# bergmanlab/TELR

Hardware: AMD Instinct MI355X
Metric: gbp_aligned_per_s (higher is better)
Workload: dtype int16

## Files before the change

telr_amd/csrc/kernels.hip.h:

```cpp
#pragma once
#include <hip/hip_runtime.h>
#include <stdint.h>

#define TELR_NEG      (-(1 << 28))
#include "part_plan.h"
#define SK_TILE       1024
#define SK_THREADS    256
#define DP_DMAX       4096

struct ChainOpt {
    int32_t max_gap, bw, min_cnt, min_chain_score, chain_gap_q8, chain_skip_q8;
    int32_t dense_n, dense_span, mw_n;
};
struct DpOpt {
    int32_t a, b, q, e, q2, e2, sc_ambi, zdrop;
    int32_t cx_scale, cx_open, cx_emax, cx_emin, cx_dec, cx_flat;
};
__host__ __device__ __forceinline__ int d_cx_ext(const DpOpt &o, int len) { int v = o.cx_emax - o.cx_dec * len; return v > o.cx_emin ? v : o.cx_emin; }
__host__ __device__ __forceinline__ int d_cx_cost(const DpOpt &o, int L)
{
    int t = o.cx_open;
    for (int i = 0; i < L && i < o.cx_flat; ++i) t += d_cx_ext(o, i);
    if (L > o.cx_flat) t += (L - o.cx_flat) * o.cx_emin;
    return t;
// ... 367 lines not shown
            const int x = __ffsll((long long)f) - 1; f &= f - 1;
            s_code[o] = (uint8_t)d_chunk_base(C, x); s_start[o] = (uint32_t)(p0 + x); ++o;
        }
    }
    __syncthreads();
    const int n = o_end - o_first;
    for (int z = threadIdx.x; z < n; z += 128) { hstart[o_first + z] = s_start[z]; hcode[o_first + z] = s_code[z]; }
}
__global__ void k_hpc_seq_offsets(const int64_t *__restrict__ boff, int32_t sid0, int32_t nseq, int64_t chunk0, const int32_t *__restrict__ coff,
                                  int32_t nchunk, int32_t total, int32_t *__restrict__ hoff )
{
    const int s = blockIdx.x * blockDim.x + threadIdx.x;
    if (s > nseq) return;
    if (s == nseq) { hoff[s] = total; return; }
    const int64_t c = boff[sid0 + s] / 64 - chunk0;
    hoff[s] = c < nchunk ? coff[c] : total;
}

struct SketchHpcArgs {
    const uint8_t *hcode; const uint32_t *hstart;
    const int32_t *hoff;
    const int32_t *len;
    const uint32_t *goff;
    const int32_t *tile_seq, *tile_u0;
    int32_t k, w;
    int32_t *tile_cnt; const int32_t *tile_off;
    uint64_t *out_x; uint32_t *out_y;
};

template <int MODE>
__global__ void __launch_bounds__(SK_THREADS) k_sketch_hpc(SketchHpcArgs A)
{
    extern __shared__ __align__(16) unsigned char smem[];
    const int halo = A.w - 1, nslot = SK_TILE + 2 * halo, k = A.k;
    uint64_t *xs = (uint64_t*)smem;
    uint32_t *ps = (uint32_t*)(xs + nslot);
    uint8_t *cb = (uint8_t*)(ps + nslot);
    uint32_t *cw = (uint32_t*)(cb + ((nslot + k - 1 + 3) & ~3)), *cn = cw + (nslot + k - 1 + 15) / 16 + 3;
    __shared__ int32_t wsum[SK_THREADS / 64];
    const int t = blockIdx.x, tid = threadIdx.x;
    const int sid = A.tile_seq[t], u0 = A.tile_u0[t];
    const int h0 = A.hoff[sid], nh = A.hoff[sid + 1] - h0, ns = nh - k + 1, L = A.len[sid];
    const uint64_t mask = (1ULL << 2 * k) - 1;
    const int lo = u0 - halo;
    for (int s = tid; s < nslot + k - 1; s += SK_THREADS) { int r = lo + s; cb[s] = (r >= 0 && r < nh) ? A.hcode[h0 + r] : 4; }
    __syncthreads();
    const int ncode = nslot + k - 1;
    for (int wq = tid; wq < (ncode + 15) / 16 + 3; wq += SK_THREADS) {
        uint32_t v = 0;
        for (int z = 0; z < 16; ++z) { const int q = wq * 16 + z; if (q < ncode) v |= (uint32_t)(cb[q] & 3) << (2 * z); }
        cw[wq] = v;
    }
    for (int wq = tid; wq < (ncode + 31) / 32 + 2; wq += SK_THREADS) {
        uint32_t v = 0;
        for (int z = 0; z < 32; ++z) { const int q = wq * 32 + z; if (q >= ncode || cb[q] > 3) v |= 1u << z; }
        cn[wq] = v;
    }
    __syncthreads();
    for (int s = tid; s < nslot; s += SK_THREADS) {
        const int u = lo + s;
        uint64_t x = UINT64_MAX; uint32_t pz = 0;
        if (u >= 0 && u < ns) {
            const int wi = s >> 4, sh = (s & 15) * 2;
            const uint64_t lo64 = (uint64_t)cw[wi] | (uint64_t)cw[wi + 1] << 32, hi64 = cw[wi + 2];
            uint64_t v = lo64 >> sh;
            if (sh) v |= hi64 << (64 - sh);
            v &= mask;
            const uint64_t nb = (((uint64_t)cn[s >> 5] | (uint64_t)cn[(s >> 5) + 1] << 32) >> (s & 31)) & ((1ULL << k) - 1);
            const bool ok = nb == 0;
            const uint64_t fw = d_rev2(v, k), rv = (~v) & mask;
            const uint32_t first = A.hstart[h0 + u];
            const uint32_t last = (u + k < nh ? A.hstart[h0 + u + k] : (uint32_t)L) - 1;
            const uint32_t span = last - first + 1;
            if (ok && fw != rv && span < 256) {
                const uint32_t z = fw < rv ? 0 : 1;
                x = d_hash64(z ? rv : fw, mask) << 8 | (uint64_t)span;
                pz = last << 1 | z;
            }
        }
        xs[s] = x; ps[s] = pz;
    }
    __syncthreads();
    const int need = A.w < ns ? A.w : ns;
    uint32_t sel = 0;
#pragma unroll
    for (int c = 0; c < SK_TILE / SK_THREADS; ++c) {
        int s = halo + tid * (SK_TILE / SK_THREADS) + c, u = lo + s;
        uint64_t x = xs[s];
        const bool is_mz = halo == 9 ? d_mz_selected<9, uint64_t>(xs, s, u, ns, need, halo, x) : d_mz_selected<0, uint64_t>(xs, s, u, ns, need, halo, x);
        if (u < ns && x != UINT64_MAX && is_mz) sel |= 1u << c;
    }
    int cnt = __popc(sel);
    int lane = tid & 63, wv = tid >> 6, inc = cnt;
#pragma unroll
    for (int o = 1; o < 64; o <<= 1) { int v = __shfl_up(inc, o); if (lane >= o) inc += v; }
    if (lane == 63) wsum[wv] = inc;
    __syncthreads();
    int wbase = 0, total = 0;
#pragma unroll
    for (int i = 0; i < SK_THREADS / 64; ++i) { if (i < wv) wbase += wsum[i]; total += wsum[i]; }
    if (MODE == 0 || MODE == 2) {
        if (tid == 0) A.tile_cnt[t] = total;
    }
    if (MODE != 0) {
        int64_t o = (MODE == 2 ? (int64_t)t * SK_TILE : (int64_t)A.tile_off[t]) + wbase + inc - cnt;
        const uint32_t g0 = A.goff ? A.goff[sid] : 0u;
#pragma unroll
        for (int c = 0; c < SK_TILE / SK_THREADS; ++c) if (sel >> c & 1) {
            int s = halo + tid * (SK_TILE / SK_THREADS) + c;
            A.out_x[o] = xs[s];
            A.out_y[o] = ((g0 << 1) + ps[s]);
            ++o;
        }
    }
}

__global__ void __launch_bounds__(256) k_ix_hash_keys(const uint64_t *__restrict__ x, const uint32_t *__restrict__ y, int64_t n, uint64_t *__restrict__ key, uint32_t *__restrict__ val)
{
    const int64_t i = (int64_t)blockIdx.x * blockDim.x + threadIdx.x;
    if (i >= n) return;
    key[i] = x[i] >> 8;
    if (val != y) val[i] = y[i];
}
__global__ void k_head_flags(const uint64_t *__restrict__ h, int64_t n, int32_t *__restrict__ flag)
{
    int64_t i = (int64_t)blockIdx.x * blockDim.x + threadIdx.x;
    if (i < n) flag[i] = (i == 0 || h[i] != h[i - 1]) ? 1 : 0;
}
__global__ void k_write_entries(const uint64_t *__restrict__ h, const int32_t *__restrict__ flag, const int32_t *__restrict__ rank,
                                int64_t n, uint64_t *__restrict__ ent_hash, uint32_t *__restrict__ ent_off, int32_t n_ent)
{
    int64_t i = (int64_t)blockIdx.x * blockDim.x + threadIdx.x;
    if (i < n && flag[i]) { ent_hash[rank[i]] = h[i]; ent_off[rank[i]] = (uint32_t)i; }
    if (i == 0) ent_off[n_ent] = (uint32_t)n;
}
__global__ void k_ent_counts(const uint32_t *__restrict__ ent_off, int32_t n_ent, uint32_t *__restrict__ cnt)
{
    int32_t i = blockIdx.x * blockDim.x + threadIdx.x;
    if (i < n_ent) cnt[i] = ent_off[i + 1] - ent_off[i];
}
__device__ __forceinline__ uint32_t d_ht_slot(uint64_t h, int ht_shift, uint32_t ht_mask)
{
    return (uint32_t)((h * 0x9E3779B97F4A7C15ULL) >> ht_shift) & ht_mask;
}
#ifndef HT_FB_LOG
#define HT_FB_LOG 1
#endif
__device__ __forceinline__ uint32_t d_ht_filter_bit(uint64_t h, int ht_shift) { return (uint32_t)((h * 0x9E3779B97F4A7C15ULL) >> (ht_shift - HT_FB_LOG)); }
struct HtSlot { uint64_t hash; uint32_t off, cnt; };
#define HT_EMPTY 0xffffffffffffffffULL
struct IndexView {
    const uint64_t *ent_hash; const uint32_t *ent_off; const uint32_t *pos; const uint32_t *bstart;
    const uint32_t *goff; const int32_t *tlen;
    int32_t n_ent; int32_t shift; int32_t k, w;
    const HtSlot *ht; int32_t ht_shift; uint32_t ht_mask;
    const uint32_t *ht_home;
};
__global__ void k_ht_build(const uint64_t *__restrict__ ent_hash, const uint32_t *__restrict__ ent_off, int32_t n_ent, int ht_shift, uint32_t ht_mask, HtSlot *__restrict__ ht,
                           uint32_t *__restrict__ ht_home, const uint32_t *__restrict__ pos)
{
    const int e = blockIdx.x * blockDim.x + threadIdx.x;
    if (e >= n_ent) return;
    const uint64_t h = ent_hash[e];
    uint32_t s = d_ht_slot(h, ht_shift, ht_mask);
    { const uint32_t f = d_ht_filter_bit(h, ht_shift); atomicOr(&ht_home[f >> 5], 1u << (f & 31)); }
    for (;;) {
        const unsigned long long old = atomicCAS((unsigned long long*)&ht[s].hash, (unsigned long long)HT_EMPTY, (unsigned long long)h);
        if (old == HT_EMPTY) { const uint32_t c = ent_off[e + 1] - ent_off[e]; ht[s].off = c == 1 ? pos[ent_off[e]] : ent_off[e]; ht[s].cnt = c; return; }
        s = (s + 1) & ht_mask;
    }
}
template <bool FILTER = true>
__device__ __forceinline__ bool d_ht_lookup(const IndexView &I, uint64_t h, uint32_t &off, uint32_t &cnt)
{
    uint32_t s = d_ht_slot(h, I.ht_shift, I.ht_mask);
    if (FILTER) { const uint32_t f = d_ht_filter_bit(h, I.ht_shift); if (!((I.ht_home[f >> 5] >> (f & 31)) & 1u)) return false; }
    for (;;) {
        const uint4 v = *(const uint4*)&I.ht[s];
        const uint64_t hh = (uint64_t)v.y << 32 | v.x;
        if (hh == h) { off = v.z; cnt = v.w; return true; }
        if (hh == HT_EMPTY) return false;
        s = (s + 1) & I.ht_mask;
    }
}

__device__ __forceinline__ uint32_t d_wave_scan_add(uint32_t v)
{
    v += (uint32_t)__builtin_amdgcn_update_dpp(0, (int)v, 0x111, 0xf, 0xf, true);
    v += (uint32_t)__builtin_amdgcn_update_dpp(0, (int)v, 0x112, 0xf, 0xf, true);
    v += (uint32_t)__builtin_amdgcn_update_dpp(0, (int)v, 0x114, 0xf, 0xf, true);
    v += (uint32_t)__builtin_amdgcn_update_dpp(0, (int)v, 0x118, 0xf, 0xf, true);
    v += (uint32_t)__builtin_amdgcn_update_dpp(0, (int)v, 0x142, 0xa, 0xf, true);
    v += (uint32_t)__builtin_amdgcn_update_dpp(0, (int)v, 0x143, 0xc, 0xf, true);
    return v;
}

struct SeedArgs {
    IndexView I;
    const uint64_t *mz_x; const uint32_t *mz_y;
    const int32_t *q_mzoff;
    const int32_t *qlen;
    const int32_t *qtarget;
    const int32_t *q_order;
    int32_t mid_occ;
    const int32_t *tmid;
    int32_t per_target;
    int32_t n_targets;
    int32_t *mz_cnt;
    int32_t *mz_ent;
    int32_t *mz_n;
    int32_t *mz_aoff;
    int32_t *q_cnt;
    const int32_t *q_aoff;
    uint64_t *keys;
    const int32_t *tile_off, *q_tile0;
    uint64_t *lds_keys;
    int32_t rescue;
};

__device__ __forceinline__ void d_put_key(const SeedArgs &A, int64_t w, uint64_t key)
{
    if (A.lds_keys) A.lds_keys[w] = key; else A.keys[w] = key;
}
__device__ __forceinline__ int d_tid_of(const uint32_t *__restrict__ goff, int n, uint32_t g)
{
    int lo = 0, hi = n - 1;
    while (lo < hi) { const int mid = (lo + hi + 1) >> 1; if (goff[mid] <= g) lo = mid; else hi = mid - 1; }
    return lo;
}

__device__ __forceinline__ uint32_t d_occ_lower(const uint32_t *__restrict__ pos, uint32_t lo, uint32_t hi, uint32_t g)
{
    while (lo < hi) { const uint32_t mid = lo + ((hi - lo) >> 1); if ((pos[mid] >> 1) < g) lo = mid + 1; else hi = mid; }
    return lo;
}
#define SEED_RESCUE_DIST    500
#define SEED_RESCUE_MAX_OCC 4095
#define SEED_RESCUE_LIST    1024
__host__ __device__ __forceinline__ int32_t seed_rescue_k(int32_t pe, int32_t ps)
{
    return (int32_t)((1000LL * (pe - ps) + 249500LL) / 500000LL);
}
__device__ __forceinline__ int64_t d_mz_slot(const SeedArgs &A, int q, int g)
{
    if (!A.tile_off) return g;
    int lo = A.q_tile0[q], hi = A.q_tile0[q + 1] - 1;
    while (lo < hi) { const int mid = (lo + hi + 1) >> 1; if (A.tile_off[mid] <= g) lo = mid; else hi = mid - 1; }
    return (int64_t)lo * SK_TILE + (g - A.tile_off[lo]);
}
__device__ __forceinline__ uint64_t d_wave_min_u64(uint64_t v)
{
    for (int o = 32; o >= 1; o >>= 1) {
        const uint64_t u = (uint64_t)(uint32_t)__shfl_xor((int)(uint32_t)v, o) | (uint64_t)(uint32_t)__shfl_xor((int)(uint32_t)(v >> 32), o) << 32;
        v = u < v ? u : v;
    }
    return v;
}
__device__ __forceinline__ void d_seed_rescue(const SeedArgs &A, const int q, const int m0, const int m1, int32_t *__restrict__ mark, const int tid, const int nthr)
{
    __shared__ int32_t s_start[SEED_RESCUE_LIST];
    __shared__ int32_t s_nstart;
    const int32_t *__restrict__ occ = A.mz_n;
    const int32_t cut = A.mid_occ;
    const int lane = tid & 63, wv = __builtin_amdgcn_readfirstlane(tid >> 6), nwv = nthr >> 6;
    const int qlen = A.qlen[q];
    for (int gb = m0; gb < m1; gb += nthr) {
        if (tid == 0) s_nstart = 0;
        __syncthreads();
        const int g = gb + tid;
        if (g < m1 && occ[g] > cut && (g == m0 || occ[g - 1] <= cut)) s_start[atomicAdd(&s_nstart, 1)] = g;
        __syncthreads();
        const int ns = s_nstart;
        for (int si = wv; si < ns; si += nwv) {
            const int s = s_start[si];
            int e = s + 1;
            for (;;) {
                const int j = e + lane;
                const uint64_t stop = __ballot(j >= m1 || occ[j < m1 ? j : m1 - 1] <= cut);
                if (stop) { e += __builtin_ctzll(stop); break; }
                e += 64;
            }
            if (e > m1) e = m1;
            const int32_t ps = s > m0 ? (int32_t)(A.mz_y[d_mz_slot(A, q, s - 1)] >> 1) : 0;
            const int32_t pe = e < m1 ? (int32_t)(A.mz_y[d_mz_slot(A, q, e)] >> 1) : qlen;
            const int32_t k = seed_rescue_k(pe, ps);
            uint64_t last = 0; bool first = true;
            for (int z = 0; z < k; ++z) {
                uint64_t best = ~0ULL;
                for (int j = s + lane; j < e; j += 64) {
                    const int32_t c = occ[j];
                    const uint64_t key = (uint64_t)(uint32_t)c << 32 | (uint32_t)(j - s);
                    if (c < SEED_RESCUE_MAX_OCC && (first || key > last) && key < best) best = key;
                }
                best = d_wave_min_u64(best);
                if (best == ~0ULL) break;
                if (lane == 0) mark[s + (int32_t)(uint32_t)best] = (int32_t)(best >> 32);
                last = best; first = false;
            }
        }
        __syncthreads();
    }
}

template <int MODE>
__device__ __forceinline__ void d_seed_query(const SeedArgs &A, const int q, const int tid, const int nthr)
{
    const int m0 = A.q_mzoff[q], m1 = A.q_mzoff[q + 1];
    const int tf = A.qtarget ? A.qtarget[q] : -1;
    const bool pt = tf < 0 && A.per_target && A.tmid;
    uint32_t g0 = 0, g1 = 0xffffffffu;
    if (tf >= 0) { g0 = A.I.goff[tf]; g1 = g0 + (uint32_t)A.I.tlen[tf]; }
    const int32_t occ = (tf >= 0 && A.tmid) ? A.tmid[tf] : A.mid_occ;
    const int qlen = A.qlen[q];
    int t = A.tile_off ? A.q_tile0[q] : 0, t_lo = 0, t_hi = 0;
    if (A.tile_off) { t_lo = A.tile_off[t]; t_hi = A.tile_off[t + 1]; }
    const int64_t wbase = MODE == 1 && !A.lds_keys ? A.q_aoff[q] : 0;
    __shared__ int32_t s_wtot[16];
    int32_t carry = 0;
    for (int gb = m0; gb < m1; gb += nthr) {
      int32_t cnt_out = 0;
      const int g = gb + tid;
      if (g < m1) do {
        int64_t gi = g;
        if (A.tile_off) {
            while (g >= t_hi) { ++t; t_lo = t_hi; t_hi = A.tile_off[t + 1]; }
            gi = (int64_t)t * SK_TILE + (g - t_lo);
        }
        uint64_t x = A.mz_x[gi];
        uint32_t o0 = 0, o1 = 0;
        if (MODE == 0) {
            uint32_t off = 0, n = 0;
            if (!d_ht_lookup(A.I, x >> 8, off, n)) n = 0;
            A.mz_ent[g] = (int32_t)off; A.mz_n[g] = (int32_t)n;
            o0 = off; o1 = off + n;
        } else {
            if (A.mz_cnt[g] == 0) break;
            o0 = (uint32_t)A.mz_ent[g]; o1 = o0 + (uint32_t)A.mz_n[g];
        }
        const bool single = o1 - o0 == 1u;
        const uint32_t pos1 = o0;
#define SEED_POS(i_) (single ? pos1 : A.I.pos[i_])
        if (pt) {
            int32_t total = 0; int64_t w = MODE == 1 ? wbase + A.mz_aoff[g] : 0;
            uint64_t kf = 0, kr = 0; int32_t qz = 0;
            if (MODE == 1) {
                const uint32_t y = A.mz_y[gi];
                const int32_t span = (int32_t)(x & 0xff), qpos = (int32_t)(y >> 1); qz = (int32_t)(y & 1);
                kf = (uint64_t)qpos << 8 | (uint64_t)span;
                kr = (1ULL << 63) | (uint64_t)(qlen - (qpos + 1 - span) - 1) << 8 | (uint64_t)span;
            }
            uint32_t o = o0;
            while (o < o1) {
                const int t = d_tid_of(A.I.goff, A.n_targets, SEED_POS(o) >> 1);
                const uint32_t gend = A.I.goff[t + 1];
                uint32_t e = o + 1;
                for (int lin = 0; e < o1 && (SEED_POS(e) >> 1) < gend; ) { ++e; if (++lin == 8) { e = d_occ_lower(A.I.pos, e, o1, gend); break; } }
                if ((int32_t)(e - o) <= A.tmid[t]) {
                    total += (int32_t)(e - o);
                    if (MODE == 1) for (uint32_t z = o; z < e; ++z) { const uint32_t py = SEED_POS(z); d_put_key(A, w++, ((int)(py & 1) == qz ? kf : kr) | (uint64_t)(py >> 1) << 32); }
                }
                o = e;
            }
            cnt_out = total;
            break;
        }
        int32_t cnt = 0;
        uint32_t a0 = o0, a1 = o1;
        if (o1 > o0) {
            if (tf >= 0) {
                if (single) { const uint32_t gp = pos1 >> 1; if (gp < g0 || gp >= g1) a1 = a0; }
                else { a0 = d_occ_lower(A.I.pos, o0, o1, g0); a1 = d_occ_lower(A.I.pos, a0, o1, g1); }
            }
            cnt = (int32_t)(a1 - a0);
            if (cnt > occ && !(MODE == 1 && A.rescue && tf < 0)) cnt = 0;
        }
        cnt_out = cnt;
        if (MODE == 1 && cnt > 0) {
            uint32_t y = A.mz_y[gi];
            int32_t span = (int32_t)(x & 0xff), qpos = (int32_t)(y >> 1), qz = (int32_t)(y & 1);
            uint64_t kf = (uint64_t)qpos << 8 | (uint64_t)span;
            uint64_t kr = (1ULL << 63) | (uint64_t)(qlen - (qpos + 1 - span) - 1) << 8 | (uint64_t)span;
            int64_t w = wbase + A.mz_aoff[g];
            for (uint32_t o = a0; o < a1; ++o) {
                const uint32_t py = SEED_POS(o);
                d_put_key(A, w++, ((int)(py & 1) == qz ? kf : kr) | (uint64_t)(py >> 1) << 32);
            }
        }
      } while (0);
      if (MODE == 0 && g < m1) A.mz_cnt[g] = cnt_out;
    }
    if (MODE == 0) {
        __syncthreads();
        if constexpr (MODE == 0) { if (A.rescue && tf < 0) { d_seed_rescue(A, q, m0, m1, A.mz_cnt, tid, nthr); __syncthreads(); } }
        const int wv = tid >> 6, nwv = (nthr + 63) >> 6;
        for (int gb = m0; gb < m1; gb += nthr) {
            const int g = gb + tid;
            const int32_t c = g < m1 ? A.mz_cnt[g] : 0;
            const uint32_t inc = d_wave_scan_add((uint32_t)c);
            if ((tid & 63) == 63) s_wtot[wv] = (int32_t)inc;
            __syncthreads();
            int32_t before = 0, all = 0;
            for (int z = 0; z < nwv; ++z) { const int32_t v = s_wtot[z]; if (z < wv) before += v; all += v; }
            if (g < m1) A.mz_aoff[g] = carry + before + (int32_t)inc - c;
            carry += all;
            __syncthreads();
        }
        if (tid == 0) A.q_cnt[q] = carry;
    }
}
#undef SEED_POS
template <int MODE>
__global__ void __launch_bounds__(256) k_seed(SeedArgs A)
{
    d_seed_query<MODE>(A, A.q_order ? A.q_order[blockIdx.x] : blockIdx.x, threadIdx.x, blockDim.x);
}

#define VOTE_SLOTS   2048
#define VOTE_SUBCAP  512
#ifndef VOTE_WAVES
#define VOTE_WAVES   3
#endif
#ifndef VOTE_HCAP
#define VOTE_HCAP    768
#endif
#define VOTE_MZ      128
struct VoteOpt { int32_t len, shift, vmin, frac_q8; };
struct VoteArgs {
    const int64_t *q_soff;
    uint64_t *stage;
    int32_t *q_cnt;
};
__device__ __forceinline__ uint32_t d_vote_slot(uint32_t gp, uint32_t qadj, uint32_t rev, int shift)
{
    const uint32_t d = gp - qadj + (1u << 24);
    return (((d >> shift) & (VOTE_SLOTS / 2 - 1)) << 1) | rev;
}
template <bool FILTER>
__global__ void __launch_bounds__(256) k_vote_lookup(IndexView I, const uint64_t *__restrict__ mz_x, int32_t nmz, int32_t mid_occ, int32_t *__restrict__ mz_ent, int32_t *__restrict__ mz_n, int32_t rescue)
{
    const int g = blockIdx.x * 256 + threadIdx.x;
    if (g >= nmz) return;
    uint32_t off = 0, n = 0;
    if (!d_ht_lookup<FILTER>(I, mz_x[g] >> 8, off, n)) n = 0;
    if (n > (uint32_t)mid_occ && !rescue) n = 0;
    mz_ent[g] = (int32_t)off; mz_n[g] = (int32_t)n;
}
__global__ void __launch_bounds__(256) k_vote_rescue(SeedArgs A)
{
    const int q = blockIdx.x, tid = threadIdx.x;
    const int m0 = A.q_mzoff[q], m1 = A.q_mzoff[q + 1];
    for (int g = m0 + tid; g < m1; g += 256) A.mz_cnt[g] = 0;
    __syncthreads();
    d_seed_rescue(A, q, m0, m1, A.mz_cnt, tid, 256);
    __syncthreads();
    for (int g = m0 + tid; g < m1; g += 256) if (A.mz_n[g] > A.mid_occ) A.mz_n[g] = A.mz_cnt[g];
}
__global__ void __launch_bounds__(64) k_vote_qhits(const int32_t *__restrict__ q_mzoff, const int32_t *__restrict__ mz_n, int32_t nq, int64_t *__restrict__ q_hits)
{
    const int q = blockIdx.x, lane = threadIdx.x;
    if (q > nq) return;
    int64_t s = 0;
    if (q < nq) for (int g = q_mzoff[q] + lane; g < q_mzoff[q + 1]; g += 64) s += mz_n[g];
    for (int o = 32; o >= 1; o >>= 1) s += (int64_t)((uint64_t)(uint32_t)__shfl_xor((int)(uint32_t)s, o) | (uint64_t)(uint32_t)__shfl_xor((int)(uint32_t)((uint64_t)s >> 32), o) << 32);
    if (lane == 0) q_hits[q] = s;
}
#ifndef VOTE_WIN
#define VOTE_WIN 8
#endif
struct VoteChunk { uint32_t P[VOTE_MZ], off[VOTE_MZ], qpos[VOTE_MZ]; uint16_t zs[VOTE_MZ]; uint8_t rid[VOTE_MZ]; uint32_t wm[2 * VOTE_WIN]; };
struct VoteHit { uint32_t gp; uint32_t sm; };
template <bool T16> __device__ __forceinline__ uint32_t d_vt_add(uint32_t *T, uint32_t s)
{
    if (T16) { const uint32_t sh = (s & 1u) << 4; return ((atomicAdd(&T[s >> 1], 1u << sh) >> sh) & 0xffffu) + 1u; }
    return atomicAdd(&T[s], 1u) + 1u;
}
template <bool T16> __device__ __forceinline__ void d_vt_vote(uint32_t *T, uint32_t s)
{
    if (T16) (void)__hip_atomic_fetch_add(&T[s >> 1], 1u << ((s & 1u) << 4), __ATOMIC_RELAXED, __HIP_MEMORY_SCOPE_WORKGROUP);
    else (void)__hip_atomic_fetch_add(&T[s], 1u, __ATOMIC_RELAXED, __HIP_MEMORY_SCOPE_WORKGROUP);
}
template <bool T16> __device__ __forceinline__ uint32_t d_vt_get(const uint32_t *T, uint32_t s)
{
    return T16 ? (T[s >> 1] >> ((s & 1u) << 4)) & 0xffffu : T[s];
}
template <bool T16>
__global__ void __launch_bounds__(64 * VOTE_WAVES) k_seed_vote(SeedArgs A, VoteOpt V, VoteArgs VA, int64_t lim16)
{
    constexpr int TW = T16 ? VOTE_SLOTS / 2 : VOTE_SLOTS;
    {
        const int q_ = A.q_order ? A.q_order[blockIdx.x] : blockIdx.x;
        const bool small = VA.q_soff[q_ + 1] - VA.q_soff[q_] <= lim16;
        if (small != T16) return;
    }
    __shared__ uint32_t tab[VOTE_WAVES][TW];
    __shared__ VoteHit stash[VOTE_WAVES][VOTE_HCAP];
    __shared__ VoteChunk chunk[VOTE_WAVES];
    __shared__ int32_t sub_first[VOTE_SUBCAP + 1];
    __shared__ uint32_t blk_cnt;
    const int q = A.q_order ? A.q_order[blockIdx.x] : blockIdx.x;
    const int m0 = A.q_mzoff[q], m1 = A.q_mzoff[q + 1];
    const int qlen = A.qlen[q];
    const int tid = threadIdx.x, lane = tid & 63, wv = __builtin_amdgcn_readfirstlane(tid >> 6);
    uint32_t *T = tab[wv];
    VoteHit *HS = stash[wv];
    VoteChunk &C = chunk[wv];
    uint64_t *out = VA.stage + VA.q_soff[q];
    for (int i = lane; i < TW; i += 64) T[i] = 0;
    if (tid == 0) blk_cnt = 0;
    const int nsub = (qlen + V.len - 1) / V.len;
    for (int sb = 0; sb < nsub; sb += VOTE_SUBCAP) {
        __syncthreads();
        for (int i = tid; i <= VOTE_SUBCAP; i += 64 * VOTE_WAVES) sub_first[i] = m1;
        __syncthreads();
        for (int g = m0 + tid; g < m1; g += 64 * VOTE_WAVES) {
            const int s = (int)(A.mz_y[g] >> 1) / V.len;
            const int sp = g > m0 ? (int)(A.mz_y[g - 1] >> 1) / V.len : -1;
            if (s != sp) {
                int lo = sp + 1 > sb ? sp + 1 : sb, hi = s < sb + VOTE_SUBCAP ? s : sb + VOTE_SUBCAP;
                for (int j = lo; j <= hi; ++j) sub_first[j - sb] = g;
            }
        }
        __syncthreads();
        const int send = nsub < sb + VOTE_SUBCAP ? nsub : sb + VOTE_SUBCAP;
        uint32_t pf_off[2] = {0, 0}, pf_n[2] = {0, 0}, pf_y[2] = {0, 0}, pf_sp[2] = {0, 0}; int pf_s = -1;
#define VOTE_LOAD_CHUNK(o_, n_, y_, sp_, gc_, g1_) { _Pragma("unroll") for (int u = 0; u < 2; ++u) { const int g = (gc_) + 2 * lane + u; o_[u] = 0; n_[u] = 0; y_[u] = 0; sp_[u] = 0; \
            if (g < (g1_)) { o_[u] = (uint32_t)A.mz_ent[g]; n_[u] = (uint32_t)A.mz_n[g]; y_[u] = A.mz_y[g]; sp_[u] = ((const uint32_t*)A.mz_x)[2 * (size_t)g]; } } }
#define VOTE_PIN(o_, n_, y_, sp_) { _Pragma("unroll") for (int u = 0; u < 2; ++u) asm volatile("" : "+v"(o_[u]), "+v"(n_[u]), "+v"(y_[u]), "+v"(sp_[u])); }
        for (int s = sb + wv; s < send; s += VOTE_WAVES) {
            const int g0 = __builtin_amdgcn_readfirstlane(sub_first[s - sb]), g1 = __builtin_amdgcn_readfirstlane(sub_first[s - sb + 1]);
            uint32_t c0_off[2], c0_n[2], c0_y[2], c0_sp[2];
            if (pf_s == s) {
                VOTE_PIN(pf_off, pf_n, pf_y, pf_sp)
#pragma unroll
                for (int u = 0; u < 2; ++u) { c0_off[u] = pf_off[u]; c0_n[u] = pf_n[u]; c0_y[u] = pf_y[u]; c0_sp[u] = pf_sp[u]; }
            } else VOTE_LOAD_CHUNK(c0_off, c0_n, c0_y, c0_sp, g0, g1)
            if (s + VOTE_WAVES < send) { pf_s = s + VOTE_WAVES; const int pg0 = __builtin_amdgcn_readfirstlane(sub_first[pf_s - sb]), pg1 = __builtin_amdgcn_readfirstlane(sub_first[pf_s - sb + 1]); VOTE_LOAD_CHUNK(pf_off, pf_n, pf_y, pf_sp, pg0, pg1) }
            if (g0 >= g1) continue;
            uint32_t vmax = 0, nhit = 0;
            for (int pass = 0; pass < 2; ++pass) {
                if (pass == 1 && nhit <= VOTE_HCAP) break;
                uint32_t thr1 = 0;
                if (pass == 1) { thr1 = (vmax * (uint32_t)V.frac_q8 + 255u) >> 8; if (thr1 < (uint32_t)V.vmin) thr1 = (uint32_t)V.vmin; }
                uint32_t hbase = 0;
                for (int gc = g0; gc < g1; gc += VOTE_MZ) {
                    uint32_t n2[2];
                    __builtin_amdgcn_wave_barrier();
                    uint32_t c_off[2], c_y[2], c_sp[2];
                    if (gc == g0) {
#pragma unroll
                        for (int u = 0; u < 2; ++u) { c_off[u] = c0_off[u]; n2[u] = c0_n[u]; c_y[u] = c0_y[u]; c_sp[u] = c0_sp[u]; }
                    } else VOTE_LOAD_CHUNK(c_off, n2, c_y, c_sp, gc, g1)
#pragma unroll
                    for (int u = 0; u < 2; ++u) { C.qpos[2 * lane + u] = c_y[u] >> 1; C.zs[2 * lane + u] = (uint16_t)((c_y[u] & 1u) << 8 | (c_sp[u] & 0xffu)); }
                    uint32_t inc = n2[0] + n2[1];
                    inc = d_wave_scan_add(inc);
                    const uint64_t nz0 = __ballot(n2[0] > 0), nz1 = __ballot(n2[1] > 0);
                    const uint64_t below = (1ULL << lane) - 1ULL;
                    const uint32_t rk0 = (uint32_t)__popcll(nz0 & below) + (uint32_t)__popcll(nz1 & below);
                    if (n2[0]) { C.rid[rk0] = (uint8_t)(2 * lane); C.P[rk0] = inc - n2[1]; C.off[rk0] = c_off[0]; }
                    if (n2[1]) { const uint32_t rk1 = rk0 + (n2[0] ? 1u : 0u); C.rid[rk1] = (uint8_t)(2 * lane + 1); C.P[rk1] = inc; C.off[rk1] = c_off[1]; }
                    const uint32_t st0 = inc - n2[0] - n2[1], st1 = inc - n2[1];
                    uint32_t cb = 0;
                    __builtin_amdgcn_wave_barrier();
                    const uint32_t H = (uint32_t)__builtin_amdgcn_readlane((int)inc, 63);
                    for (uint32_t h0 = 0; h0 < H; h0 += 64 * VOTE_WIN) {
                        uint32_t m_[VOTE_WIN], py_[VOTE_WIN]; bool in_[VOTE_WIN];
                        if (lane < 2 * VOTE_WIN) C.wm[lane] = 0;
                        __builtin_amdgcn_wave_barrier();
                        { const uint32_t d0 = st0 - h0, d1 = st1 - h0;
                          if (n2[0] && d0 < 64u * VOTE_WIN) atomicOr(&C.wm[d0 >> 5], 1u << (d0 & 31));
                          if (n2[1] && d1 < 64u * VOTE_WIN) atomicOr(&C.wm[d1 >> 5], 1u << (d1 & 31)); }
                        __builtin_amdgcn_wave_barrier();
#pragma unroll
                        for (int u = 0; u < VOTE_WIN; ++u) {
                            const uint32_t h = h0 + 64 * u + lane;
                            in_[u] = h < H; m_[u] = 0; py_[u] = 0;
                            if (h0 + 64 * u < H) {
                                const uint64_t wmask = (uint64_t)C.wm[2 * u + 1] << 32 | C.wm[2 * u];
                                const uint32_t upto = (uint32_t)__popcll(wmask & ((2ULL << lane) - 1ULL));
                                if (in_[u]) {
                                    const uint32_t r = cb + upto - 1u;
                                    const uint32_t pm = r ? C.P[r - 1] : 0u, nm = C.P[r] - pm, of = C.off[r];
                                    m_[u] = C.rid[r];
                                    py_[u] = nm == 1 ? of : A.I.pos[of + (h - pm)];
                                }
                                cb += (uint32_t)__popcll(wmask);
                            }
                        }
#pragma unroll
                        for (int u = 0; u < VOTE_WIN; ++u) {
                            if (h0 + 64 * u >= H) break;
                            const uint32_t h = h0 + 64 * u + lane;
                            bool pass_hit = false; uint32_t gp_ = 0, rv_ = 0;
                            if (in_[u]) {
                                const uint32_t m = m_[u], zs = C.zs[m], span = zs & 0xffu, qpos = C.qpos[m];
                                rv_ = (py_[u] & 1u) ^ (zs >> 8); gp_ = py_[u] >> 1;
                                const uint32_t qadj = rv_ ? (uint32_t)qlen - (qpos + 1 - span) - 1 : qpos;
                                const uint32_t sl_ = d_vote_slot(gp_, qadj, rv_, V.shift);
                                if (pass == 0) {
                                    d_vt_vote<T16>(T, sl_);
                                    if (hbase + h < VOTE_HCAP) { VoteHit x; x.gp = gp_; x.sm = sl_ | m << 11 | (uint32_t)(gc - g0) / VOTE_MZ << 18; HS[hbase + h] = x; }
                                } else pass_hit = d_vt_get<T16>(T, (sl_ - 2u) & (VOTE_SLOTS - 1)) + d_vt_get<T16>(T, sl_) + d_vt_get<T16>(T, (sl_ + 2u) & (VOTE_SLOTS - 1)) >= thr1;
                            }
                            if (pass == 1) {
                                const uint64_t bm = __ballot(pass_hit);
                                uint32_t base = 0;
                                if (lane == 0 && bm) base = atomicAdd(&blk_cnt, (uint32_t)__popcll(bm));
                                base = (uint32_t)__shfl((int)base, 0);
                                if (pass_hit) {
                                    const uint32_t m = m_[u], zs = C.zs[m], span = zs & 0xffu, qpos = C.qpos[m];
                                    const uint64_t key = (rv_ ? (1ULL << 63) | (uint64_t)((uint32_t)qlen - (qpos + 1 - span) - 1) << 8 : (uint64_t)qpos << 8) | (uint64_t)span | (uint64_t)gp_ << 32;
                                    out[base + (uint32_t)__popcll(bm & ((1ULL << lane) - 1ULL))] = key;
                                }
                            }
                        }
                    }
                    hbase += H;
                }
                if (pass == 0) {
                    nhit = hbase;
                    if (nhit > VOTE_HCAP) {
                        __builtin_amdgcn_wave_barrier();
                        for (int i = lane; i < TW; i += 64) { const uint32_t w_ = T[i]; const uint32_t a_ = T16 ? (w_ & 0xffffu) : w_, b_ = T16 ? (w_ >> 16) : 0u; vmax = a_ > vmax ? a_ : vmax; vmax = b_ > vmax ? b_ : vmax; }
                        for (int o = 32; o >= 1; o >>= 1) { const uint32_t v = (uint32_t)__shfl_xor((int)vmax, o); vmax = v > vmax ? v : vmax; }
                    }
                }
            }
            __builtin_amdgcn_wave_barrier();
            const bool one_chunk = g1 - g0 <= VOTE_MZ;
            if (nhit <= VOTE_HCAP) {
                constexpr int NG = VOTE_HCAP / 64;
                VoteHit xs[NG]; uint32_t s3[NG]; uint32_t cmax = 0;
#pragma unroll
                for (int g = 0; g < NG; ++g) {
                    xs[g].gp = 0; xs[g].sm = 0; s3[g] = 0;
                    if ((uint32_t)(g * 64) < nhit) {
                        const uint32_t h = (uint32_t)(g * 64) + lane;
                        if (h < nhit) {
                            xs[g] = HS[h];
                            const uint32_t sl = xs[g].sm & (VOTE_SLOTS - 1);
                            const uint32_t c_ = d_vt_get<T16>(T, sl);
                            s3[g] = d_vt_get<T16>(T, (sl - 2u) & (VOTE_SLOTS - 1)) + c_ + d_vt_get<T16>(T, (sl + 2u) & (VOTE_SLOTS - 1));
                            cmax = c_ > cmax ? c_ : cmax;
                        }
                    }
                }
                for (int o = 32; o >= 1; o >>= 1) { const uint32_t v = (uint32_t)__shfl_xor((int)cmax, o); cmax = v > cmax ? v : cmax; }
                vmax = cmax;
                uint32_t thr = (vmax * (uint32_t)V.frac_q8 + 255u) >> 8;
                if (thr < (uint32_t)V.vmin) thr = (uint32_t)V.vmin;
                uint64_t bm[NG]; uint32_t tot = 0;
#pragma unroll
                for (int g = 0; g < NG; ++g) {
                    bm[g] = 0;
                    if ((uint32_t)(g * 64) < nhit) { bm[g] = __ballot((uint32_t)(g * 64) + lane < nhit && s3[g] >= thr); tot += (uint32_t)__popcll(bm[g]); }
                }
                uint32_t base = 0;
                if (lane == 0 && tot) base = atomicAdd(&blk_cnt, tot);
                base = (uint32_t)__shfl((int)base, 0);
#pragma unroll
                for (int g = 0; g < NG; ++g) {
                    if ((uint32_t)(g * 64) < nhit) {
                        if ((bm[g] >> lane) & 1ULL) {
                            const VoteHit x = xs[g];
                            const uint32_t mi = (x.sm >> 11) & (VOTE_MZ - 1);
                            uint32_t span, qpos;
                            if (one_chunk) { span = C.zs[mi] & 0xffu; qpos = C.qpos[mi]; }
                            else { const int gq = g0 + (int)(x.sm >> 18) * VOTE_MZ + (int)mi; span = (uint32_t)(A.mz_x[gq] & 0xff); qpos = A.mz_y[gq] >> 1; }
                            const uint32_t rev = x.sm & 1u;
                            const uint64_t key = (rev ? (1ULL << 63) | (uint64_t)((uint32_t)qlen - (qpos + 1 - span) - 1) << 8 : (uint64_t)qpos << 8) | (uint64_t)span | (uint64_t)x.gp << 32;
                            out[base + (uint32_t)__popcll(bm[g] & ((1ULL << lane) - 1ULL))] = key;
                        }
                        base += (uint32_t)__popcll(bm[g]);
                    }
                }
                __builtin_amdgcn_wave_barrier();
                for (uint32_t h = lane; h < nhit; h += 64) { const uint32_t sl = HS[h].sm & (VOTE_SLOTS - 1); T[T16 ? sl >> 1 : sl] = 0; }
            } else for (int i = lane; i < TW; i += 64) T[i] = 0;
            __builtin_amdgcn_wave_barrier();
        }
    }
    __syncthreads();
    if (tid == 0) VA.q_cnt[q] = (int32_t)blk_cnt;
}
#undef VOTE_LOAD_CHUNK
#undef VOTE_PIN
__global__ void __launch_bounds__(256) k_vote_compact(const uint64_t *__restrict__ stage, const int64_t *__restrict__ q_soff, const int32_t *__restrict__ q_aoff, int32_t nq,
                                                      uint64_t *__restrict__ keys)
{
    if ((int)blockIdx.x >= nq) return;
    const int q = (int)blockIdx.x;
    const int64_t s0 = q_soff[q]; const int a0 = q_aoff[q], n = q_aoff[q + 1] - a0;
// ... 2683 lines not shown
```

Baseline: 21.19.

## Batch seed probes per thread in emit pass to overlap independent loads

In the key-emitting pass, each thread now handles several minimizers per iteration (SEED_PROBE_BATCH, default 4). It issues all count, entry, position and offset loads up front, resolves tile indices through a prefetched window of tile offsets, and gathers index positions in groups of four before writing keys. The aim is to expose memory-level parallelism and hide the latency of dependent global loads. The cost is higher register pressure, which may lower occupancy, plus extra clamped loads that are wasted on inactive slots.

```diff
diff --git a/telr_amd/csrc/kernels.hip.h b/telr_amd/csrc/kernels.hip.h
--- a/telr_amd/csrc/kernels.hip.h
+++ b/telr_amd/csrc/kernels.hip.h
@@ -693,9 +693,17 @@
     }
 }
 
+#ifndef SEED_PROBE_BATCH
+#define SEED_PROBE_BATCH 4
+#endif
+#define SEED_ARRIVED(v_) asm volatile("" : "+v"(v_))
+#define SEED_TILE_WIN 8
 template <int MODE>
 __device__ __forceinline__ void d_seed_query(const SeedArgs &A, const int q, const int tid, const int nthr)
 {
+    constexpr int U = MODE == 1 ? SEED_PROBE_BATCH : 1;
+    constexpr int OG = U > 1 ? 4 : 1;
+    static_assert(U >= 1 && U <= 8, "SEED_PROBE_BATCH");
     const int m0 = A.q_mzoff[q], m1 = A.q_mzoff[q + 1];
     const int tf = A.qtarget ? A.qtarget[q] : -1;
     const bool pt = tf < 0 && A.per_target && A.tmid;
@@ -705,47 +713,86 @@
     const int qlen = A.qlen[q];
     int t = A.tile_off ? A.q_tile0[q] : 0, t_lo = 0, t_hi = 0;
     if (A.tile_off) { t_lo = A.tile_off[t]; t_hi = A.tile_off[t + 1]; }
+    const int t_end = A.tile_off && U > 1 ? A.q_tile0[q + 1] : 0;
     const int64_t wbase = MODE == 1 && !A.lds_keys ? A.q_aoff[q] : 0;
     __shared__ int32_t s_wtot[16];
     int32_t carry = 0;
-    for (int gb = m0; gb < m1; gb += nthr) {
+    for (int gb = m0; gb + tid < m1; gb += U * nthr) {
+      int g[U]; bool live[U]; int64_t gi[U];
+#pragma unroll
+      for (int u = 0; u < U; ++u) { g[u] = gb + tid + u * nthr; live[u] = g[u] < m1; gi[u] = live[u] ? g[u] : g[0]; }
+      if (A.tile_off) {
+        if constexpr (U == 1) {
+            while (g[0] >= t_hi) { ++t; t_lo = t_hi; t_hi = A.tile_off[t + 1]; }
+            gi[0] = (int64_t)t * SK_TILE + (g[0] - t_lo);
+        } else {
+            int32_t nxt[SEED_TILE_WIN];
+#pragma unroll
+            for (int j = 0; j < SEED_TILE_WIN; ++j) nxt[j] = A.tile_off[min(t + 2 + j, t_end)];
+            int tu = t, lo = t_lo, hi = t_hi;
+#pragma unroll
+            for (int u = 0; u < U; ++u) {
+                if (live[u]) {
+                    tu = t; lo = t_lo; hi = t_hi;
+#pragma unroll
+                    for (int j = 0; j < SEED_TILE_WIN; ++j) if (g[u] >= hi) { ++tu; lo = hi; hi = nxt[j]; }
+                    while (g[u] >= hi) { ++tu; lo = hi; hi = A.tile_off[tu + 1]; }
+                    gi[u] = (int64_t)tu * SK_TILE + (g[u] - lo);
+                } else gi[u] = gi[0];
+            }
+            t = tu; t_lo = lo; t_hi = hi;
+        }
+      }
+      uint64_t x[U]; uint32_t o0[U], o1[U]; uint32_t y[U]; int32_t aoff[U];
+#pragma unroll
+      for (int u = 0; u < U; ++u) { x[u] = 0; o0[u] = o1[u] = 0; y[u] = 0; aoff[u] = 0; }
+      if (MODE == 0) {
+        x[0] = A.mz_x[gi[0]];
+        uint32_t off = 0, n = 0;
+        if (!d_ht_lookup(A.I, x[0] >> 8, off, n)) n = 0;
+        A.mz_ent[g[0]] = (int32_t)off; A.mz_n[g[0]] = (int32_t)n;
+        o0[0] = off; o1[0] = off + n;
+      } else {
+        int32_t c[U];
+#pragma unroll
+        for (int u = 0; u < U; ++u) c[u] = A.mz_cnt[live[u] ? g[u] : g[0]];
+#pragma unroll
+        for (int u = 0; u < U; ++u) SEED_ARRIVED(c[u]);
+#pragma unroll
+        for (int u = 0; u < U; ++u) live[u] = live[u] && c[u] != 0;
+#pragma unroll
+        for (int u = 0; u < U; ++u) {
+            if (live[u]) {
+                x[u] = A.mz_x[gi[u]];
+                o0[u] = (uint32_t)A.mz_ent[g[u]]; o1[u] = (uint32_t)A.mz_n[g[u]];
+                if (U > 1) { y[u] = A.mz_y[gi[u]]; aoff[u] = A.mz_aoff[g[u]]; }
+            }
+        }
+#pragma unroll
+        for (int u = 0; u < U; ++u) o1[u] += o0[u];
+      }
+#pragma unroll
+      for (int u = 0; u < U; ++u) {
       int32_t cnt_out = 0;
-      const int g = gb + tid;
-      if (g < m1) do {
-        int64_t gi = g;
-        if (A.tile_off) {
-            while (g >= t_hi) { ++t; t_lo = t_hi; t_hi = A.tile_off[t + 1]; }
-            gi = (int64_t)t * SK_TILE + (g - t_lo);
-        }
-        uint64_t x = A.mz_x[gi];
-        uint32_t o0 = 0, o1 = 0;
-        if (MODE == 0) {
-            uint32_t off = 0, n = 0;
-            if (!d_ht_lookup(A.I, x >> 8, off, n)) n = 0;
-            A.mz_ent[g] = (int32_t)off; A.mz_n[g] = (int32_t)n;
-            o0 = off; o1 = off + n;
-        } else {
-            if (A.mz_cnt[g] == 0) break;
-            o0 = (uint32_t)A.mz_ent[g]; o1 = o0 + (uint32_t)A.mz_n[g];
-        }
-        const bool single = o1 - o0 == 1u;
-        const uint32_t pos1 = o0;
+      if (live[u]) do {
+        const bool single = o1[u] - o0[u] == 1u;
+        const uint32_t pos1 = o0[u];
 #define SEED_POS(i_) (single ? pos1 : A.I.pos[i_])
         if (pt) {
-            int32_t total = 0; int64_t w = MODE == 1 ? wbase + A.mz_aoff[g] : 0;
+            int32_t total = 0; int64_t w = MODE == 1 ? wbase + (U > 1 ? aoff[u] : A.mz_aoff[g[u]]) : 0;
             uint64_t kf = 0, kr = 0; int32_t qz = 0;
             if (MODE == 1) {
-                const uint32_t y = A.mz_y[gi];
-                const int32_t span = (int32_t)(x & 0xff), qpos = (int32_t)(y >> 1); qz = (int32_t)(y & 1);
+                const uint32_t yy = U > 1 ? y[u] : A.mz_y[gi[u]];
+                const int32_t span = (int32_t)(x[u] & 0xff), qpos = (int32_t)(yy >> 1); qz = (int32_t)(yy & 1);
                 kf = (uint64_t)qpos << 8 | (uint64_t)span;
                 kr = (1ULL << 63) | (uint64_t)(qlen - (qpos + 1 - span) - 1) << 8 | (uint64_t)span;
             }
-            uint32_t o = o0;
-            while (o < o1) {
+            uint32_t o = o0[u];
+            while (o < o1[u]) {
                 const int t = d_tid_of(A.I.goff, A.n_targets, SEED_POS(o) >> 1);
                 const uint32_t gend = A.I.goff[t + 1];
                 uint32_t e = o + 1;
-                for (int lin = 0; e < o1 && (SEED_POS(e) >> 1) < gend; ) { ++e; if (++lin == 8) { e = d_occ_lower(A.I.pos, e, o1, gend); break; } }
+                for (int lin = 0; e < o1[u] && (SEED_POS(e) >> 1) < gend; ) { ++e; if (++lin == 8) { e = d_occ_lower(A.I.pos, e, o1[u], gend); break; } }
                 if ((int32_t)(e - o) <= A.tmid[t]) {
                     total += (int32_t)(e - o);
                     if (MODE == 1) for (uint32_t z = o; z < e; ++z) { const uint32_t py = SEED_POS(z); d_put_key(A, w++, ((int)(py & 1) == qz ? kf : kr) | (uint64_t)(py >> 1) << 32); }
@@ -756,29 +803,33 @@
             break;
         }
         int32_t cnt = 0;
-        uint32_t a0 = o0, a1 = o1;
-        if (o1 > o0) {
+        uint32_t a0 = o0[u], a1 = o1[u];
+        if (o1[u] > o0[u]) {
             if (tf >= 0) {
                 if (single) { const uint32_t gp = pos1 >> 1; if (gp < g0 || gp >= g1) a1 = a0; }
-                else { a0 = d_occ_lower(A.I.pos, o0, o1, g0); a1 = d_occ_lower(A.I.pos, a0, o1, g1); }
+                else { a0 = d_occ_lower(A.I.pos, o0[u], o1[u], g0); a1 = d_occ_lower(A.I.pos, a0, o1[u], g1); }
             }
             cnt = (int32_t)(a1 - a0);
             if (cnt > occ && !(MODE == 1 && A.rescue && tf < 0)) cnt = 0;
         }
         cnt_out = cnt;
         if (MODE == 1 && cnt > 0) {
-            uint32_t y = A.mz_y[gi];
-            int32_t span = (int32_t)(x & 0xff), qpos = (int32_t)(y >> 1), qz = (int32_t)(y & 1);
+            const uint32_t yy = U > 1 ? y[u] : A.mz_y[gi[u]];
+            int32_t span = (int32_t)(x[u] & 0xff), qpos = (int32_t)(yy >> 1), qz = (int32_t)(yy & 1);
             uint64_t kf = (uint64_t)qpos << 8 | (uint64_t)span;
             uint64_t kr = (1ULL << 63) | (uint64_t)(qlen - (qpos + 1 - span) - 1) << 8 | (uint64_t)span;
-            int64_t w = wbase + A.mz_aoff[g];
-            for (uint32_t o = a0; o < a1; ++o) {
-                const uint32_t py = SEED_POS(o);
-                d_put_key(A, w++, ((int)(py & 1) == qz ? kf : kr) | (uint64_t)(py >> 1) << 32);
+            int64_t w = wbase + (U > 1 ? aoff[u] : A.mz_aoff[g[u]]);
+            for (uint32_t o = a0; o < a1; o += OG, w += OG) {
+                uint32_t py[OG];
+#pragma unroll
+                for (int j = 0; j < OG; ++j) py[j] = SEED_POS(min(o + (uint32_t)j, a1 - 1u));
+#pragma unroll
+                for (int j = 0; j < OG; ++j) if (o + (uint32_t)j < a1) d_put_key(A, w + j, ((int)(py[j] & 1) == qz ? kf : kr) | (uint64_t)(py[j] >> 1) << 32);
             }
         }
       } while (0);
-      if (MODE == 0 && g < m1) A.mz_cnt[g] = cnt_out;
+      if (MODE == 0 && g[u] < m1) A.mz_cnt[g[u]] = cnt_out;
+      }
     }
     if (MODE == 0) {
         __syncthreads();
```

After: 21.83, median of 6. 1.03x the previous value.
